# cloneofsimo/paint-with-words-sd

Measured on AMD Instinct MI355X. Metric: 512x512 images/sec (30 steps, CFG) SD1.5+PwW, higher is better.
Workload: dtype bf16

## Files before the change

### include/pww_hip_linear.h

```cpp
#ifndef PWW_HIP_LINEAR_H
#define PWW_HIP_LINEAR_H

#include "pww_hip.h"

#ifdef __cplusplus
extern "C" {
#endif

#define PWW_LINEAR_VERSION 100

int pww_linear_version(void);
const char *pww_linear_last_error(void);

#define PWW_LINEAR_NONE 0
#define PWW_LINEAR_BIAS 1
#define PWW_LINEAR_BIAS_RESIDUAL 2
#define PWW_LINEAR_BIAS_GEGLU 3
typedef struct pww_linear_desc {
    uint32_t size;
    int32_t dtype;
    int32_t M, N, K;
    int32_t epilogue;
    int64_t x_stride, y_stride, r_stride;
    int32_t tile_n, splitk;
} pww_linear_desc_t;
size_t pww_linear_workspace_bytes(const pww_linear_desc_t *desc);
int pww_linear_fwd(const void *x, const void *w, const void *bias, const void *residual, void *y, const pww_linear_desc_t *desc, void *workspace,
                   size_t workspace_bytes, void *stream);

#ifdef __cplusplus
}
#endif

#endif
```

### paint-with-words-sd_amd/build.py

```python
import os
import subprocess
import sys

HERE = os.path.dirname(os.path.abspath(__file__))
REPO = os.path.dirname(HERE)
CSRC = os.path.join(HERE, "csrc")
LIB = os.path.join(HERE, "pww_hip", "libpww_hip.so")
LIB_EXPERIMENTS = os.path.join(HERE, "pww_hip", "libpww_hip_experiments.so")
UNITS = [("pww_api.hip", [], ""), ("pww_attn.hip", [], ""), ("pww_cross.hip", [], ""), ("pww_cross_lean.hip", [], ""), ("pww_reduce.hip", [], ""),
         ("pww_mask.hip", [], ""), ("pww_qproj.hip", [], ""), ("pww_norm.hip", [], ""), ("pww_blocks.hip", [], ""), ("pww_conv.hip", [], ""), ("pww_probs.hip", [], ""),
         ("pww_attn_inst.hip", ["-DPWW_INST_F16"], ".f16"), ("pww_attn_inst.hip", ["-DPWW_INST_BF16"], ".bf16"),
         ("pww_cross_inst.hip", ["-DPWW_INST_F16", "-DPWW_INST_NW=2"], ".f16.nw2"), ("pww_cross_inst.hip", ["-DPWW_INST_F16", "-DPWW_INST_NW=4"], ".f16.nw4"),
         ("pww_cross_inst.hip", ["-DPWW_INST_BF16", "-DPWW_INST_NW=2"], ".bf16.nw2"), ("pww_cross_inst.hip", ["-DPWW_INST_BF16", "-DPWW_INST_NW=4"], ".bf16.nw4")]
EXPERIMENT_UNITS = [("pww_cross_out.hip", [], "")]
_ATTN_HEADERS = ["pww_tile.h", "pww_attn_core.h", "pww_cross_tile.h"]
SIDE_FLAGS = ["-fvisibility=hidden"]
SIDE_LIBS = {
    "long": ("pww_long.hip", _ATTN_HEADERS, "the long-prompt launches"),
    "scope": ("pww_scope.hip", _ATTN_HEADERS, "cross-attention with per-head / per-row score statistics"),
    "linear": ("pww_linear.hip", [], "linear layers with a bias / residual / GEGLU epilogue"),
    "regions": ("pww_regions.hip", [], "region masks and the per-pixel blend of the noise predictions"),
}
SOURCES = sorted({u[0] for u in UNITS + EXPERIMENT_UNITS})
HEADERS = ["pww_common.h", "pww_tile.h", "pww_attn_core.h", "pww_attn_kernel.h", "pww_cross_tile.h", "pww_cross_kernel.h", os.path.join(REPO, "include", "pww_hip.h")]
LIB_LONG, LIB_SCOPE, LIB_LINEAR, LIB_REGIONS = (os.path.join(HERE, "pww_hip", "libpww_hip_%s.so" % n) for n in SIDE_LIBS)
LONG_UNITS, SCOPE_UNITS, LINEAR_UNITS, REGIONS_UNITS = ([(v[0], SIDE_FLAGS, "")] for v in SIDE_LIBS.values())
HIPCC = os.environ.get("HIPCC", "/opt/rocm/bin/hipcc")
FLAGS = ["--offload-arch=gfx950", "-O3", "-std=c++17", "-fPIC", "-Wall",
         "-Wno-unused-function", "-mllvm", "-amdgpu-kernarg-preload-count=16"]


PER_FILE_FLAGS = {"pww_mask.hip": ["-ffp-contract=off"], "pww_regions.hip": ["-ffp-contract=off"]}


def _newer(target, deps):
    if not os.path.exists(target):
        return True
    t = os.path.getmtime(target)
    return any(os.path.getmtime(d) > t for d in deps)


def _deps():
    return ([os.path.join(CSRC, s) for s in SOURCES] + [h if os.path.isabs(h) else os.path.join(CSRC, h) for h in HEADERS] + [__file__])


def _build(lib, units, defines, objdir, verbose, jobs=None):
    os.makedirs(objdir, exist_ok=True)
# ... 79 lines not shown
```

### paint-with-words-sd_amd/csrc/pww_conv.hip

```cpp
#include "pww_common.h"

namespace pww {

namespace {

constexpr int CV_BM = 128, CV_THREADS = 256;
constexpr int CV_PF = 2;

__device__ __forceinline__ f32x4 mfma16(f16x8 a, f16x8 b, f32x4 c) { return __builtin_amdgcn_mfma_f32_16x16x32_f16(a, b, c, 0, 0, 0); }
__device__ __forceinline__ f32x4 mfma16(bf16x8 a, bf16x8 b, f32x4 c) { return __builtin_amdgcn_mfma_f32_16x16x32_bf16(a, b, c, 0, 0, 0); }

struct ConvCold {
    const void *bias, *residual;
    int nsplit, nslab;
};

__device__ __forceinline__ int xcd_remap(int orig, int nwg) {
    const int xcd = orig & 7, q = nwg >> 3, r = nwg & 7;
    return (xcd < r ? xcd * (q + 1) : r * (q + 1) + (xcd - r) * q) + (orig >> 3);
}

template <typename T>
__device__ __forceinline__ void epilogue4(const f32x4 &a, const ConvCold &cold, T *y, long off, int n) {
    typedef typename Vec<T>::v4 V4;
    V4 o;
#pragma unroll
    for (int j = 0; j < 4; ++j) o[j] = (T)a[j];
    if (cold.bias) {
        const V4 b = *reinterpret_cast<const V4 *>(reinterpret_cast<const T *>(cold.bias) + n);
#pragma unroll
        for (int j = 0; j < 4; ++j) o[j] = (T)((float)o[j] + (float)b[j]);
    }
    if (cold.residual) {
        const V4 r = *reinterpret_cast<const V4 *>(reinterpret_cast<const T *>(cold.residual) + off);
#pragma unroll
        for (int j = 0; j < 4; ++j) o[j] = (T)((float)r[j] + (float)o[j]);
    }
    *reinterpret_cast<V4 *>(y + off) = o;
}

template <typename T, int BN>
__global__ void __launch_bounds__(CV_THREADS, 2) conv3x3_kernel(const T *__restrict__ x, const T *__restrict__ w, void *__restrict__ out, int M, int N,
                                                            int Cin, int Hin, int Win, int Wo, int HWo, const ConvCold cold) {
    typedef typename Vec<T>::v8 V8;
    constexpr int BM = CV_BM, PF = CV_PF, XL = BM * 8 / CV_THREADS, WL = BN * 8 / CV_THREADS, RM = 4, RN = BN / 32;
    constexpr int XBYTES = BM * 128, STAGE = (BM + BN) * 128;
    __shared__ __attribute__((aligned(16))) char lds[2 * STAGE];

    const int geo = cold.nslab >> 24;
    const int nslab = cold.nslab & 0xffffff;
    const int stride = geo & 15, up = geo >> 4;
    const int Hv = Hin << up, Wv = Win << up;
    const int tid = threadIdx.x, lane = tid & 63, wave = tid >> 6, wm = wave >> 1, wn = wave & 1;
    const int ntm = (M + BM - 1) / BM;
    const int bid = xcd_remap(blockIdx.x, gridDim.x);
    const bool split = cold.nsplit > 1;
    const int tile = bid / cold.nsplit, ks = bid - tile * cold.nsplit;
    const int tm = tile % ntm, tn = tile / ntm;
    const int s_begin = (int)((long)ks * nslab / cold.nsplit), s_end = (int)((long)(ks + 1) * nslab / cold.nsplit);
    const int K9 = 9 * Cin;

// ... 90 lines not shown
        }
    }
#pragma unroll
    for (int t = 0; t < 2 * PF - 1; ++t) {
        if (i + t < n) {
            if (i + t + PF < n) load(t % PF);
            compute((i + t) & 1);
            if (i + t + 1 < n) store((t + 1) % PF, (i + t + 1) & 1);
            __syncthreads();
        }
    }

#pragma unroll
    for (int i = 0; i < RM; ++i) {
        const int m = tm * BM + wm * 64 + i * 16 + fr;
        if (m >= M) continue;
#pragma unroll
        for (int r = 0; r < RN; ++r) {
            const int n = tn * BN + wn * (BN / 2) + r * 16 + fq * 4;
            if (split) *reinterpret_cast<f32x4 *>(reinterpret_cast<float *>(out) + ((long)ks * M + m) * N + n) = acc[r][i];
            else epilogue4<T>(acc[r][i], cold, reinterpret_cast<T *>(out), (long)m * N + n, n);
        }
    }
}

template <typename T>
__global__ void __launch_bounds__(256) conv3x3_fold_kernel(const float *__restrict__ ws, T *__restrict__ y, long n4, int N, long MN, const ConvCold cold) {
    const long q = (long)blockIdx.x * 256 + threadIdx.x;
    if (q >= n4) return;
    const long off = q * 4;
    f32x4 a = *reinterpret_cast<const f32x4 *>(ws + off);
    for (int s = 1; s < cold.nsplit; ++s) a += *reinterpret_cast<const f32x4 *>(ws + s * MN + off);
    epilogue4<T>(a, cold, y, off, (int)(off % N));
}

struct ConvTune { int M, N, nslab, bn, nsplit; };
constexpr ConvTune CONV_TUNED[] = {
    {8192, 320, 45, 64, 3}, {8192, 320, 90, 64, 4}, {8192, 320, 135, 64, 3}, {8192, 640, 90, 128, 3},
    {2048, 320, 45, 64, 6}, {2048, 640, 45, 64, 3}, {2048, 640, 90, 128, 6}, {2048, 640, 135, 128, 6}, {2048, 640, 180, 128, 6},
    {2048, 640, 270, 128, 6}, {2048, 1280, 180, 128, 3},
    {512, 640, 90, 64, 6}, {512, 1280, 90, 128, 6}, {512, 1280, 180, 128, 12}, {512, 1280, 270, 128, 12}, {512, 1280, 360, 128, 12},
    {128, 1280, 180, 64, 12}, {128, 1280, 360, 64, 24},
    {65536, 640, 90, 128, 1}, {16384, 1280, 180, 128, 1},
    {4096, 640, 90, 128, 3}, {4096, 1280, 90, 128, 3}, {4096, 1280, 180, 128, 3}, {4096, 1280, 270, 128, 3}, {4096, 1280, 360, 128, 3},
    {1024, 1280, 180, 128, 6}, {1024, 1280, 360, 128, 6},
};

struct ConvPlan {
    int M, Ho, Wo, bn, nsplit, nslab, ntiles;
};

bool plan_conv(const pww_conv_desc_t *d, ConvPlan *p) {
    if (!d || d->size < sizeof(pww_conv_desc_t)) { set_error("conv3x3: descriptor missing or older than this library (size %u)", d ? d->size : 0u); return false; }
    const int up = d->upsample, s = d->stride;
    if ((d->dtype != PWW_DTYPE_F16 && d->dtype != PWW_DTYPE_BF16) || d->B < 1 || d->Hin < 1 || d->Win < 1 || d->Cin < 64 || d->Cin % 64 != 0
        || d->Cout < 64 || d->Cout % 64 != 0 || (s != 1 && s != 2) || (up != 0 && up != 1) || (up && s != 1) || d->Cin > 65536 || d->Cout > 65536) {
// ... 77 lines not shown
```

### paint-with-words-sd_amd/csrc/pww_linear.hip

```cpp
#define PWW_SIDE_LIB "libpww_hip_linear"
#include "pww_side_host.h"
#include "../../include/pww_hip_linear.h"

#define PWW_LINEAR_API extern "C" __attribute__((visibility("default")))

namespace pww {

namespace {

constexpr int LN_BM = 128, LN_THREADS = 256;
constexpr int LN_PF = 2;

__device__ __forceinline__ f32x4 mfma16(f16x8 a, f16x8 b, f32x4 c) { return __builtin_amdgcn_mfma_f32_16x16x32_f16(a, b, c, 0, 0, 0); }
__device__ __forceinline__ f32x4 mfma16(bf16x8 a, bf16x8 b, f32x4 c) { return __builtin_amdgcn_mfma_f32_16x16x32_bf16(a, b, c, 0, 0, 0); }

struct LinCold {
    const void *bias, *residual;
    long ys, rs;
    int nsplit, nslab, mode, inner;
};

__device__ __forceinline__ int xcd_remap(int orig, int nwg) {
    const int xcd = orig & 7, q = nwg >> 3, r = nwg & 7;
    return (xcd < r ? xcd * (q + 1) : r * (q + 1) + (xcd - r) * q) + (orig >> 3);
// ... 265 lines not shown
int linear_fwd(const void *x, const void *w, const void *bias, const void *residual, void *y, const pww_linear_desc_t *d, void *workspace,
               size_t workspace_bytes, hipStream_t stream) {
    LinPlan p;
    if (!plan_linear(d, &p)) return PWW_ENOTSUP;
    if (!x || !w || !y) { set_error("linear: x, w and y are required"); return PWW_EINVAL; }
    if ((d->epilogue >= PWW_LINEAR_BIAS && !bias) || (d->epilogue == PWW_LINEAR_BIAS_RESIDUAL && !residual)) {
        set_error("linear: epilogue %d needs its bias%s", d->epilogue, d->epilogue == PWW_LINEAR_BIAS_RESIDUAL ? " and residual" : "");
        return PWW_EINVAL;
    }
    if (!al16(x) || !al16(w) || !al16(y) || (reinterpret_cast<uintptr_t>(bias) & 7) || (reinterpret_cast<uintptr_t>(residual) & 7)) {
        set_error("linear: x, w, y must be 16-byte aligned, bias and residual 8-byte aligned");
        return PWW_EINVAL;
    }
    const size_t need = p.nsplit > 1 ? (size_t)p.nsplit * d->M * d->N * sizeof(float) : 0;
    if (need && (!workspace || !al16(workspace) || workspace_bytes < need)) {
        set_error("linear: split %d needs a 16-byte aligned workspace of %zu bytes (got %zu)", p.nsplit, need, workspace_bytes);
        return PWW_EINVAL;
    }
    if (!arch_ok()) return PWW_ENOTSUP;
    if (d->dtype == PWW_DTYPE_F16) return linear_launch<f16>(p, d, x, w, bias, residual, y, workspace, stream);
    return linear_launch<bf16>(p, d, x, w, bias, residual, y, workspace, stream);
}

}

PWW_LINEAR_API int pww_linear_version(void) { return PWW_LINEAR_VERSION; }
PWW_LINEAR_API const char *pww_linear_last_error(void) { return pww::last_error(); }
PWW_LINEAR_API size_t pww_linear_workspace_bytes(const pww_linear_desc_t *desc) { return pww::linear_workspace_bytes(desc); }
PWW_LINEAR_API int pww_linear_fwd(const void *x, const void *w, const void *bias, const void *residual, void *y, const pww_linear_desc_t *desc,
                                  void *workspace, size_t workspace_bytes, void *stream) {
    return pww::linear_fwd(x, w, bias, residual, y, desc, workspace, workspace_bytes, static_cast<hipStream_t>(stream));
}
```

### paint-with-words-sd_amd/pww_hip/_lib.py

```python
import ctypes
import os

_HERE = os.path.dirname(os.path.abspath(__file__))
LIB_PATH = os.environ.get("PWW_HIP_LIB", os.path.join(_HERE, "libpww_hip.so"))
EXPERIMENTS_LIB_PATH = os.environ.get("PWW_HIP_EXPERIMENTS_LIB", os.path.join(_HERE, "libpww_hip_experiments.so"))

LONG_LIB_PATH = os.environ.get("PWW_HIP_LONG_LIB", os.path.join(_HERE, "libpww_hip_long.so"))
SCOPE_LIB_PATH = os.environ.get("PWW_HIP_SCOPE_LIB", os.path.join(_HERE, "libpww_hip_scope.so"))
LINEAR_LIB_PATH = os.environ.get("PWW_HIP_LINEAR_LIB", os.path.join(_HERE, "libpww_hip_linear.so"))
REGIONS_LIB_PATH = os.environ.get("PWW_HIP_REGIONS_LIB", os.path.join(_HERE, "libpww_hip_regions.so"))

PWW_OK, PWW_EINVAL, PWW_ENOTSUP, PWW_EHIP = 0, -22, -95, -5
MIN_VERSION = 126
DTYPE_F16, DTYPE_BF16 = 0, 1
LAYOUT_NCHW, LAYOUT_NHWC = 0, 1
ACT_NONE, ACT_SILU = 0, 1
LINEAR_NONE, LINEAR_BIAS, LINEAR_BIAS_RESIDUAL, LINEAR_BIAS_GEGLU = 0, 1, 2, 3
MAX_HEAD_DIM = 160

EXPORTS = ("pww_version", "pww_has_experiments", "pww_last_error", "pww_device_arch", "pww_self_attn_fwd", "pww_cross_attn_fwd",
           "pww_cross_attn_fwd_stat", "pww_cross_attn_fwd_stat_ex",
           "pww_qk_reduce", "pww_mask_build", "pww_mask_build_rgb", "pww_mask_build_f32", "pww_resize_tokens", "pww_gauss_blur", "pww_inpaint_prep", "pww_cfg_combine", "pww_store_f32",
           "pww_workspace_bytes", "pww_profile_arm", "pww_profile_elapsed_us", "pww_profile_reset", "pww_debug_timeline", "pww_debug_path_counts",
           "pww_qproj_stat", "pww_qproj_parts", "pww_cross_attn_fwd_parts", "pww_mask_build_f32_levels", "pww_qk_parts", "pww_qk_parts_count",
           "pww_group_norm_fwd", "pww_group_norm_workspace_bytes", "pww_add_layer_norm", "pww_add_layer_norm_bias", "pww_geglu", "pww_bias_residual",
           "pww_conv3x3_workspace_bytes", "pww_conv3x3_fwd", "pww_cross_attn_probs")
EXPERIMENT_EXPORTS = ("pww_cross_attn_fwd_fused", "pww_cross_attn_fwd_fused_ex", "pww_cross_fused_workspace_bytes", "pww_cross_fused_state_bytes",
                      "pww_cross_attn_fwd_parts_out", "pww_cross_attn_out_supported")


LONG_EXPORTS = ("pww_long_version", "pww_long_last_error", "pww_long_qk_parts", "pww_long_qk_parts_count", "pww_long_cross_attn_fwd_parts",
                "pww_long_cross_attn_probs", "pww_long_profile_arm", "pww_long_profile_elapsed_us")
LONG_MIN_VERSION = 100
LONG_MIN_KEYS, LONG_MAX_KEYS = 129, 256


SCOPE_EXPORTS = ("pww_scope_version", "pww_scope_last_error", "pww_scope_head_parts_count", "pww_scope_head_parts", "pww_scope_cross_attn_fwd")
SCOPE_MIN_VERSION = 100
SCOPE_HEAD, SCOPE_ROW = 1, 2


LINEAR_EXPORTS = ("pww_linear_version", "pww_linear_last_error", "pww_linear_workspace_bytes", "pww_linear_fwd")
LINEAR_MIN_VERSION = 100


REGIONS_EXPORTS = ("pww_regions_version", "pww_regions_last_error", "pww_regions_masks", "pww_regions_combine")
REGIONS_MIN_VERSION = 100
REGIONS_MAX, REGIONS_MAX_PLANE, REGIONS_MAX_FEATHER = 8, 9216, 8.0


class AttnDesc(ctypes.Structure):
    _fields_ = [("dtype", ctypes.c_int32), ("B", ctypes.c_int32), ("H", ctypes.c_int32), ("N", ctypes.c_int32),
                ("M", ctypes.c_int32), ("D", ctypes.c_int32),
                ("q_stride", ctypes.c_int64 * 3), ("k_stride", ctypes.c_int64 * 3),
                ("v_stride", ctypes.c_int64 * 3), ("o_stride", ctypes.c_int64 * 3),
                ("scale", ctypes.c_float), ("bias_stride", ctypes.c_int64 * 4)]


class CrossOpts(ctypes.Structure):
    _fields_ = [("size", ctypes.c_uint32), ("bias_cols", ctypes.c_int32), ("coeff_scalar_dev", ctypes.c_void_p),
                ("bias_compact", ctypes.c_void_p), ("col_idx", ctypes.c_void_p), ("R", ctypes.c_int32), ("gated_images", ctypes.c_int32),
                ("compact_stride", ctypes.c_int64 * 2), ("col_idx_stride", ctypes.c_int64)]


class QprojDesc(ctypes.Structure):
# ... 161 lines not shown
    if not lib.pww_has_experiments():
        raise PwwHipError("%s was not built with -DPWW_EXPERIMENTS=1" % EXPERIMENTS_LIB_PATH)
    _exp = _bind(lib, True)
    return _exp


_P = ctypes.POINTER
_vp, _i32, _i64, _f32, _f64, _sz, _int = ctypes.c_void_p, ctypes.c_int32, ctypes.c_int64, ctypes.c_float, ctypes.c_double, ctypes.c_size_t, ctypes.c_int
_HINT = "(rebuild: python paint-with-words-sd_amd/build.py, or __graft_entry__.build())"
SIDE = {
    "long": dict(path="LONG_LIB_PATH", exports=LONG_EXPORTS, min_version=LONG_MIN_VERSION, missing_ok=False, needs="prompts longer than 77 tokens need it", sigs={
        "pww_long_qk_parts": ([_vp, _vp, _vp, _P(AttnDesc), _i32, _i32, _vp, _sz, _vp], _int),
        "pww_long_qk_parts_count": ([_P(AttnDesc)], _i32),
        "pww_long_cross_attn_fwd_parts": ([_vp, _vp, _vp, _vp, _vp, _i32, _f32, _vp, _P(AttnDesc), _vp, _i32, _vp, _P(CrossOpts), _vp], _int),
        "pww_long_cross_attn_probs": ([_vp, _vp, _vp, _vp, _i32, _f64, _f32, _vp, _P(AttnDesc), _P(CrossOpts), _vp, _P(ProbsDesc), _vp], _int),
        "pww_long_profile_arm": ([], _int),
        "pww_long_profile_elapsed_us": ([_P(_f32)], _int)}),
    "scope": dict(path="SCOPE_LIB_PATH", exports=SCOPE_EXPORTS, min_version=SCOPE_MIN_VERSION, missing_ok=True, needs="per-head / per-row score statistics need it", sigs={
        "pww_scope_head_parts_count": ([_P(AttnDesc)], _i32),
        "pww_scope_head_parts": ([_vp, _vp, _vp, _P(AttnDesc), _i32, _vp, _sz, _vp], _int),
        "pww_scope_cross_attn_fwd": ([_vp, _vp, _vp, _vp, _vp, _i32, _i32, _f32, _vp, _P(AttnDesc), _vp, _i32, _vp, _P(CrossOpts), _vp], _int)}),
    "linear": dict(path="LINEAR_LIB_PATH", exports=LINEAR_EXPORTS, min_version=LINEAR_MIN_VERSION, missing_ok=False, needs="linear layers on the native kernel need it", sigs={
        "pww_linear_workspace_bytes": ([_P(LinearDesc)], _sz),
        "pww_linear_fwd": ([_vp, _vp, _vp, _vp, _vp, _P(LinearDesc), _vp, _sz, _vp], _int)}),
    "regions": dict(path="REGIONS_LIB_PATH", exports=REGIONS_EXPORTS, min_version=REGIONS_MIN_VERSION, missing_ok=False, needs="region prompts need it", sigs={
        "pww_regions_masks": ([_vp, _i32, _i32, _vp, _i32, _f32, _vp, _vp], _int),
        "pww_regions_combine": ([_vp, _vp, _vp, _vp, _f32, _vp, _i32, _i32, _i32, _i64, _i32, _vp], _int)}),
}
_side = {}


def load_side(name):
    lib = _side.get(name)
    if lib is not None:
        return lib
    spec, path, so, pre = SIDE[name], globals()[SIDE[name]["path"]], "libpww_hip_%s.so" % name, "pww_%s_" % name
    if not os.path.isfile(path):
        if spec["missing_ok"]:
            return None
        raise PwwHipError("%s not found at %s: %s %s" % (so, path, spec["needs"], _HINT))
    try:
        lib = ctypes.CDLL(path)
        getattr(lib, pre + "version").restype = _int
        version = getattr(lib, pre + "version")()
    except (OSError, AttributeError) as e:
        raise PwwHipError("%s at %s cannot be loaded: %s %s" % (so, path, e, _HINT))
    if version // 100 != 1 or version < spec["min_version"]:
# ... 58 lines not shown
```

### paint-with-words-sd_amd/pww_hip/blocks.py

```python
import os
import types
import warnings

import torch
import torch.nn as nn
import torch.nn.functional as F

from . import ops

FUSED_NORM = os.environ.get("PWW_FUSED_NORM", "1") != "0"
BATCHED_TEMB = os.environ.get("PWW_BATCHED_TEMB", "1") != "0"
FOLD_CONV_BIAS = os.environ.get("PWW_FOLD_CONV_BIAS", "1") != "0"
CONV1X1_AS_LINEAR = os.environ.get("PWW_CONV1X1_AS_LINEAR", "1") != "0"
LINEAR = os.environ.get("PWW_LINEAR", "1")
CONV3X3 = os.environ.get("PWW_CONV3X3", "1") != "0"


_STATS = {k: [0, 0] for k in ("group_norm", "resnet_block", "transformer_block", "geglu", "conv1x1", "conv3x3", "linear")}
_UNRATED = ("conv1x1", "conv3x3", "linear")
_warned = set()


def stats():
    out = {k: {"fused": v[0], "declined": v[1]} for k, v in _STATS.items()}
    rated = [v for k, v in _STATS.items() if k not in _UNRATED]
    tot = sum(v[0] + v[1] for v in rated)
    out["hit_rate"] = (sum(v[0] for v in rated) / tot) if tot else None
    return out


def reset_stats():
    for v in _STATS.values():
        v[0] = v[1] = 0


def _count(op, fused, x=None, reason=None):
    _STATS[op][0 if fused else 1] += 1
    if not fused and FUSED_NORM and torch.is_tensor(x) and x.is_cuda and x.dtype in (torch.float16, torch.bfloat16):
# ... 89 lines not shown
        return out


def _conv_no_bias(conv, x):
    return F.conv2d(x, conv.weight, None, conv.stride, conv.padding, conv.dilation, conv.groups)


def _plain_conv(conv):
    return isinstance(conv, nn.Conv2d) and conv.bias is not None and conv.padding_mode == "zeros" and type(conv).forward is nn.Conv2d.forward \
        and "forward" not in conv.__dict__ and not conv._forward_hooks and not conv._forward_pre_hooks


def _resnet_forward(self, *args, **kwargs):
    covered = 1 <= len(args) <= 2 and set(kwargs) <= {"temb"} and not (len(args) == 2 and kwargs)
    input_tensor = args[0] if args else None
    if not covered or not _takes(input_tensor, self.norm1):
        _count("resnet_block", False, input_tensor, ("a call beyond (input_tensor, temb): %d positional, keywords %s" % (len(args), sorted(kwargs))) if not covered else _why_not(input_tensor))
        return self._pww_orig_forward(*args, **kwargs)
    temb = args[1] if len(args) == 2 else kwargs.get("temb")
    _count("resnet_block", True)
    fold = FOLD_CONV_BIAS and _plain_conv(self.conv1) and _plain_conv(self.conv2) and self.conv1.bias.dtype == input_tensor.dtype
    h = fused_group_norm(self.norm1, input_tensor, act="silu")
    if fold and _conv3x3_route(self.conv1, h):
        h = ops.conv3x3(h, self.conv1.weight)
    else:
        h = _conv_no_bias(self.conv1, h) if fold else self.conv1(h)
    add = None
    if temb is not None and getattr(self, "time_emb_proj", None) is not None:
        slot = self.__dict__.get("_pww_temb_slot")
        if slot is not None and temb.dtype == h.dtype and temb.dim() == 2 and not torch.is_grad_enabled():
            add = slot[0].project(temb)[:, slot[1]:slot[1] + slot[2]]
        else:
            add = self.time_emb_proj(F.silu(temb))
        if add.dtype != h.dtype:
            add = add.to(h.dtype)
    if fold and _takes(h, self.norm2):
        h = ops.group_norm(h, self.norm2.num_groups, self.norm2.weight, self.norm2.bias, self.norm2.eps, add=add, act="silu", pre_bias=self.conv1.bias)
    else:
        if fold:
            h = h + self.conv1.bias[None, :, None, None]
        h = fused_group_norm(self.norm2, h, add=add, act="silu")
    dropout = getattr(self, "dropout", None)
    if dropout is not None:
        h = dropout(h)
    if getattr(self, "conv_shortcut", None) is not None:
        input_tensor = self.conv_shortcut(input_tensor)
    scale = getattr(self, "output_scale_factor", 1.0)
    if fold and input_tensor.dtype == h.dtype and input_tensor.shape == (h.shape[0], self.conv2.out_channels) + h.shape[2:] and _conv3x3_route(self.conv2, h):
        out = ops.conv3x3(h, self.conv2.weight, self.conv2.bias, residual=input_tensor)
    elif fold and input_tensor.dtype == h.dtype and input_tensor.shape[1] % 8 == 0:
        out = ops.bias_residual(input_tensor, _conv_no_bias(self.conv2, h), self.conv2.bias)
    else:
        out = input_tensor + self.conv2(h)
    return out if scale == 1.0 else out / scale


def _is_conv3x3(m):
    return (isinstance(m, nn.Conv2d) and type(m).forward is nn.Conv2d.forward and m.kernel_size == (3, 3) and m.stride in ((1, 1), (2, 2))
            and m.padding == (1, 1) and m.dilation == (1, 1) and m.groups == 1 and m.padding_mode == "zeros")


STOCK_FROM_ROWS = 16384


def _conv3x3_route(conv, x, upsample=False):
    ok = (CONV3X3 and FUSED_NORM and torch.is_tensor(x) and x.dim() == 4 and _is_conv3x3(conv) and not torch.is_autocast_enabled() and not (torch.is_grad_enabled() and (x.requires_grad or conv.weight.requires_grad))
          and (conv.bias is None or conv.bias.dtype == x.dtype) and ops.conv3x3_takes(x, conv.weight, conv.stride[0], upsample)
          and (upsample or x.shape[0] * ((x.shape[2] - 1) // conv.stride[0] + 1) * ((x.shape[3] - 1) // conv.stride[0] + 1) < STOCK_FROM_ROWS))
    _STATS["conv3x3"][0 if ok else 1] += 1
    return ok


def _conv3x3_forward(self, x, *args, **kwargs):
    if not args and not kwargs and _conv3x3_route(self, x):
        return ops.conv3x3(x, self.weight, self.bias, stride=self.stride[0])
    return self._pww_orig_forward(x, *args, **kwargs)


def _upsample_conv(m):
    if getattr(m, "use_conv_transpose", False) or not getattr(m, "use_conv", True):
        return None
    conv = getattr(m, "Conv2d_0", None) if getattr(m, "name", "conv") != "conv" else getattr(m, "conv", None)
    return conv if _is_conv3x3(conv) and conv.stride == (1, 1) and "forward" not in conv.__dict__ and not conv._forward_hooks and not conv._forward_pre_hooks else None


def _upsample_forward(self, *args, **kwargs):
    plain = 1 <= len(args) <= 2 and set(kwargs) <= {"output_size"} and all(a is None for a in list(args[1:]) + list(kwargs.values()))
    x = args[0] if plain and not (len(args) == 2 and kwargs) else None
    conv = _upsample_conv(self)
    if x is not None and conv is not None and x.dim() == 4 and (getattr(self, "channels", None) in (None, x.shape[1])) and _conv3x3_route(conv, x, upsample=True):
        return ops.conv3x3(x, conv.weight, conv.bias, upsample=True)
    return self._pww_orig_forward(*args, **kwargs)


def _conv1x1_forward(self, x, *args, **kwargs):
    if (not args and not kwargs and FUSED_NORM and CONV1X1_AS_LINEAR and torch.is_tensor(x) and x.is_cuda and x.dim() == 4 and x.dtype == self.weight.dtype
            and x.shape[2] * x.shape[3] > 1 and x.is_contiguous(memory_format=torch.channels_last) and not torch.is_autocast_enabled()):
        B, C, H, W = x.shape
        _STATS["conv1x1"][0] += 1
        y = F.linear(x.permute(0, 2, 3, 1).reshape(B * H * W, C), self.weight.reshape(self.out_channels, C), self.bias)
        return y.view(B, H, W, self.out_channels).permute(0, 3, 1, 2)
    _STATS["conv1x1"][1] += 1
    return self._pww_orig_forward(x, *args, **kwargs)


def _is_conv1x1(m):
    return (isinstance(m, nn.Conv2d) and type(m).forward is nn.Conv2d.forward and m.kernel_size == (1, 1) and m.stride == (1, 1) and m.padding == (0, 0)
            and m.dilation == (1, 1) and m.groups == 1 and m.padding_mode == "zeros")


def _ln_takes(x, norm):
    return (FUSED_NORM and torch.is_tensor(x) and x.is_cuda and x.dtype in (torch.float16, torch.bfloat16) and x.dim() >= 2
            and len(norm.normalized_shape) == 1 and x.shape[-1] == norm.normalized_shape[0] and x.shape[-1] % 8 == 0 and x.shape[-1] <= 2048
            and (norm.weight is None or norm.weight.dtype == x.dtype) and not torch.is_autocast_enabled()
# ... 126 lines not shown
```

### paint-with-words-sd_amd/pww_hip/ops.py

```python
import ctypes

import torch

from . import _lib
from ._lib import AttnDesc, CrossOpts, ProbsDesc, QprojDesc, Region, PwwHipError

_DT = {torch.float16: _lib.DTYPE_F16, torch.bfloat16: _lib.DTYPE_BF16}


def _stream():
    return ctypes.c_void_p(torch.cuda.current_stream().cuda_stream)


def _ptr(t):
    return ctypes.c_void_p(t.data_ptr()) if t is not None else ctypes.c_void_p(0)


def _require_gpu(*tensors):
    for t in tensors:
        if t is not None and not t.is_cuda:
            raise PwwHipError("pww_hip ops need tensors on a HIP device (got %s); there is no CPU path" % t.device)


def _rows_ok(t):
# ... 888 lines not shown

def _khwc_weight(weight):
    if weight.is_contiguous(memory_format=torch.channels_last):
        return weight
    key = (weight.data_ptr(), weight._version, weight.dtype, weight.device)
    hit = weight.__dict__.get("_pww_khwc")
    if hit is not None and hit[0] == key:
        return hit[1]
    packed = weight.detach().permute(0, 2, 3, 1).contiguous()
    weight.__dict__["_pww_khwc"] = (key, packed)
    return packed


def conv3x3_takes(x, weight, stride=1, upsample=False):
    if not (torch.is_tensor(x) and x.is_cuda and x.dim() == 4 and x.dtype in _DT and torch.is_tensor(weight) and weight.dtype == x.dtype and weight.dim() == 4):
        return False
    B, C, H, W = x.shape
    Cout = weight.shape[0]
    return (tuple(weight.shape[1:]) == (C, 3, 3) and C % 64 == 0 and Cout % 64 == 0 and stride in (1, 2) and not (upsample and stride != 1)
            and x.is_contiguous(memory_format=torch.channels_last) and x.data_ptr() % 16 == 0
            and B * H * W * C < 2 ** 31 // 4)


def conv3x3(x, weight, bias=None, residual=None, stride=1, upsample=False, tile_n=0, splitk=0):
    _require_gpu(x, weight, bias, residual)
    if not conv3x3_takes(x, weight, stride, upsample):
        raise PwwHipError("conv3x3: needs a channels_last float16/bfloat16 x with Cin, Cout multiples of 64 and a 3 x 3 weight of its dtype")
    B, C, H, W = x.shape
    Cout = weight.shape[0]
    Hv, Wv = H << int(bool(upsample)), W << int(bool(upsample))
    Ho, Wo = (Hv - 1) // stride + 1, (Wv - 1) // stride + 1
    w = _khwc_weight(weight)
    if bias is not None and (bias.dtype != x.dtype or tuple(bias.shape) != (Cout,)):
        raise PwwHipError("conv3x3: bias must be a %s [%d]" % (x.dtype, Cout))
    if bias is not None:
        bias = bias.contiguous()
    if residual is not None:
        if tuple(residual.shape) != (B, Cout, Ho, Wo) or residual.dtype != x.dtype:
            raise PwwHipError("conv3x3: residual must be a %s %s" % (x.dtype, (B, Cout, Ho, Wo)))
        residual = residual.contiguous(memory_format=torch.channels_last)
    d = _lib.ConvDesc(ctypes.sizeof(_lib.ConvDesc), _DT[x.dtype], B, H, W, C, Cout, int(stride), int(bool(upsample)), int(tile_n), int(splitk), 0)
    lib = _lib.load()
    y = torch.empty((B, Cout, Ho, Wo), dtype=x.dtype, device=x.device, memory_format=torch.channels_last)
    nbytes = int(lib.pww_conv3x3_workspace_bytes(ctypes.byref(d)))
    ws = torch.empty(nbytes // 4, dtype=torch.float32, device=x.device) if nbytes else None
    with torch.cuda.device(x.device):
        _lib.check(lib.pww_conv3x3_fwd(_ptr(x), _ptr(w), _ptr(bias), _ptr(residual), _ptr(y), ctypes.byref(d), _ptr(ws), nbytes, _stream()), "pww_conv3x3_fwd")
    return y


def _linear_weight(weight):
    if not torch.is_tensor(weight) or weight.dim() not in (2, 4) or (weight.dim() == 4 and tuple(weight.shape[2:]) != (1, 1)):
        return None
    w = weight.detach().reshape(weight.shape[0], weight.shape[1]) if weight.dim() == 4 else weight.detach()
    return w if w.is_contiguous() and w.data_ptr() == weight.data_ptr() and w.data_ptr() % 16 == 0 else None


def linear_takes(x, weight, geglu=False, bias=None, residual=None, out=None):
    if not (torch.is_tensor(x) and x.is_cuda and x.dtype in _DT and x.dim() >= 2 and torch.is_tensor(weight) and weight.dtype == x.dtype):
        return False
    w = _linear_weight(weight)
    if w is None or x.shape[-1] != w.shape[1] or x.numel() == 0 or _rows(x, "linear") is None:
        return False
    N, K = w.shape
    rows, _, xs = _rows(x, "linear")
    if not (K % 64 == 0 and N % (128 if geglu else 64) == 0 and rows * xs < 2 ** 31 and rows * N < 2 ** 31 and N * K < 2 ** 31):
# ... 52 lines not shown
```

Measured before the change: 5.132.

## Add staged-row 3x3 convolution kernel reusing input rows across kx taps

Adds a new implicit-GEMM 3x3 conv kernel that stages a tile of 128+2 input pixel rows in LDS once per (ky, channel-block) and reuses it for all three kx taps, zeroing the left and right image edges in registers. Only the weights are reloaded per tap, which is meant to cut global input traffic and address math compared with the existing conv kernel. It comes with per-shape tuned tile widths and split-K factors, and is routed for the listed stride-1 SD1.5 UNet shapes. Upsample and stride-2 convs keep the old kernel. Adds code in the linear side library and a fallback path when the new kernel reports it is unsupported.

Measured after the change: 5.215, median of 6. 1.02x the previous value.

```diff
diff --git a/include/pww_hip_linear.h b/include/pww_hip_linear.h
--- a/include/pww_hip_linear.h
+++ b/include/pww_hip_linear.h
@@ -28,6 +28,18 @@
 int pww_linear_fwd(const void *x, const void *w, const void *bias, const void *residual, void *y, const pww_linear_desc_t *desc, void *workspace,
                    size_t workspace_bytes, void *stream);
 
+typedef struct pww_linear_conv_desc {
+    uint32_t size;
+    int32_t dtype;
+    int32_t B, Hin, Win, Cin, Cout;
+    int32_t stride, upsample;
+    int32_t tile_n, splitk;
+    int32_t _pad;
+} pww_linear_conv_desc_t;
+size_t pww_linear_conv3x3_workspace_bytes(const pww_linear_conv_desc_t *desc);
+int pww_linear_conv3x3_fwd(const void *x, const void *w, const void *bias, const void *residual, void *y, const pww_linear_conv_desc_t *desc,
+                           void *workspace, size_t workspace_bytes, void *stream);
+
 #ifdef __cplusplus
 }
 #endif
diff --git a/paint-with-words-sd_amd/build.py b/paint-with-words-sd_amd/build.py
--- a/paint-with-words-sd_amd/build.py
+++ b/paint-with-words-sd_amd/build.py
@@ -18,11 +18,11 @@
 SIDE_LIBS = {
     "long": ("pww_long.hip", _ATTN_HEADERS, "the long-prompt launches"),
     "scope": ("pww_scope.hip", _ATTN_HEADERS, "cross-attention with per-head / per-row score statistics"),
-    "linear": ("pww_linear.hip", [], "linear layers with a bias / residual / GEGLU epilogue"),
+    "linear": ("pww_linear.hip", ["pww_conv_rows.h", "pww_conv_fold.h"], "linear layers with a bias / residual / GEGLU epilogue; the staged-row 3 x 3 convolution"),
     "regions": ("pww_regions.hip", [], "region masks and the per-pixel blend of the noise predictions"),
 }
 SOURCES = sorted({u[0] for u in UNITS + EXPERIMENT_UNITS})
-HEADERS = ["pww_common.h", "pww_tile.h", "pww_attn_core.h", "pww_attn_kernel.h", "pww_cross_tile.h", "pww_cross_kernel.h", os.path.join(REPO, "include", "pww_hip.h")]
+HEADERS = ["pww_common.h", "pww_conv_fold.h", "pww_tile.h", "pww_attn_core.h", "pww_attn_kernel.h", "pww_cross_tile.h", "pww_cross_kernel.h", os.path.join(REPO, "include", "pww_hip.h")]
 LIB_LONG, LIB_SCOPE, LIB_LINEAR, LIB_REGIONS = (os.path.join(HERE, "pww_hip", "libpww_hip_%s.so" % n) for n in SIDE_LIBS)
 LONG_UNITS, SCOPE_UNITS, LINEAR_UNITS, REGIONS_UNITS = ([(v[0], SIDE_FLAGS, "")] for v in SIDE_LIBS.values())
 HIPCC = os.environ.get("HIPCC", "/opt/rocm/bin/hipcc")
diff --git a/paint-with-words-sd_amd/csrc/pww_conv.hip b/paint-with-words-sd_amd/csrc/pww_conv.hip
--- a/paint-with-words-sd_amd/csrc/pww_conv.hip
+++ b/paint-with-words-sd_amd/csrc/pww_conv.hip
@@ -10,33 +10,11 @@
 __device__ __forceinline__ f32x4 mfma16(f16x8 a, f16x8 b, f32x4 c) { return __builtin_amdgcn_mfma_f32_16x16x32_f16(a, b, c, 0, 0, 0); }
 __device__ __forceinline__ f32x4 mfma16(bf16x8 a, bf16x8 b, f32x4 c) { return __builtin_amdgcn_mfma_f32_16x16x32_bf16(a, b, c, 0, 0, 0); }
 
-struct ConvCold {
-    const void *bias, *residual;
-    int nsplit, nslab;
-};
+#include "pww_conv_fold.h"
 
 __device__ __forceinline__ int xcd_remap(int orig, int nwg) {
     const int xcd = orig & 7, q = nwg >> 3, r = nwg & 7;
     return (xcd < r ? xcd * (q + 1) : r * (q + 1) + (xcd - r) * q) + (orig >> 3);
-}
-
-template <typename T>
-__device__ __forceinline__ void epilogue4(const f32x4 &a, const ConvCold &cold, T *y, long off, int n) {
-    typedef typename Vec<T>::v4 V4;
-    V4 o;
-#pragma unroll
-    for (int j = 0; j < 4; ++j) o[j] = (T)a[j];
-    if (cold.bias) {
-        const V4 b = *reinterpret_cast<const V4 *>(reinterpret_cast<const T *>(cold.bias) + n);
-#pragma unroll
-        for (int j = 0; j < 4; ++j) o[j] = (T)((float)o[j] + (float)b[j]);
-    }
-    if (cold.residual) {
-        const V4 r = *reinterpret_cast<const V4 *>(reinterpret_cast<const T *>(cold.residual) + off);
-#pragma unroll
-        for (int j = 0; j < 4; ++j) o[j] = (T)((float)r[j] + (float)o[j]);
-    }
-    *reinterpret_cast<V4 *>(y + off) = o;
 }
 
 template <typename T, int BN>
@@ -173,16 +151,6 @@
             else epilogue4<T>(acc[r][i], cold, reinterpret_cast<T *>(out), (long)m * N + n, n);
         }
     }
-}
-
-template <typename T>
-__global__ void __launch_bounds__(256) conv3x3_fold_kernel(const float *__restrict__ ws, T *__restrict__ y, long n4, int N, long MN, const ConvCold cold) {
-    const long q = (long)blockIdx.x * 256 + threadIdx.x;
-    if (q >= n4) return;
-    const long off = q * 4;
-    f32x4 a = *reinterpret_cast<const f32x4 *>(ws + off);
-    for (int s = 1; s < cold.nsplit; ++s) a += *reinterpret_cast<const f32x4 *>(ws + s * MN + off);
-    epilogue4<T>(a, cold, y, off, (int)(off % N));
 }
 
 struct ConvTune { int M, N, nslab, bn, nsplit; };
diff --git a/paint-with-words-sd_amd/csrc/pww_conv_fold.h b/paint-with-words-sd_amd/csrc/pww_conv_fold.h
--- /dev/null
+++ b/paint-with-words-sd_amd/csrc/pww_conv_fold.h
@@ -0,0 +1,35 @@
+#pragma once
+
+struct ConvCold {
+    const void *bias, *residual;
+    int nsplit, nslab;
+};
+
+template <typename T>
+__device__ __forceinline__ void epilogue4(const f32x4 &a, const ConvCold &cold, T *y, long off, int n) {
+    typedef typename Vec<T>::v4 V4;
+    V4 o;
+#pragma unroll
+    for (int j = 0; j < 4; ++j) o[j] = (T)a[j];
+    if (cold.bias) {
+        const V4 b = *reinterpret_cast<const V4 *>(reinterpret_cast<const T *>(cold.bias) + n);
+#pragma unroll
+        for (int j = 0; j < 4; ++j) o[j] = (T)((float)o[j] + (float)b[j]);
+    }
+    if (cold.residual) {
+        const V4 r = *reinterpret_cast<const V4 *>(reinterpret_cast<const T *>(cold.residual) + off);
+#pragma unroll
+        for (int j = 0; j < 4; ++j) o[j] = (T)((float)r[j] + (float)o[j]);
+    }
+    *reinterpret_cast<V4 *>(y + off) = o;
+}
+
+template <typename T>
+__global__ void __launch_bounds__(256) conv3x3_fold_kernel(const float *__restrict__ ws, T *__restrict__ y, long n4, int N, long MN, const ConvCold cold) {
+    const long q = (long)blockIdx.x * 256 + threadIdx.x;
+    if (q >= n4) return;
+    const long off = q * 4;
+    f32x4 a = *reinterpret_cast<const f32x4 *>(ws + off);
+    for (int s = 1; s < cold.nsplit; ++s) a += *reinterpret_cast<const f32x4 *>(ws + s * MN + off);
+    epilogue4<T>(a, cold, y, off, (int)(off % N));
+}
diff --git a/paint-with-words-sd_amd/csrc/pww_conv_rows.h b/paint-with-words-sd_amd/csrc/pww_conv_rows.h
--- /dev/null
+++ b/paint-with-words-sd_amd/csrc/pww_conv_rows.h
@@ -0,0 +1,161 @@
+#pragma once
+#include "pww_conv_fold.h"
+
+constexpr int CR_BM = 128, CR_THREADS = 256, CR_XROWS = CR_BM + 2;
+
+template <typename T, int BN>
+__global__ void __launch_bounds__(CR_THREADS, 2) conv3x3_rows_kernel(const T *__restrict__ x, const T *__restrict__ w, void *__restrict__ out, int M, int N,
+                                                                     int Cin, int H, int W, const ConvCold cold) {
+    typedef typename Vec<T>::v8 V8;
+    constexpr int BM = CR_BM, XL = BM * 8 / CR_THREADS + 1, WL = BN * 8 / CR_THREADS, RM = 4, RN = BN / 32;
+    constexpr int XIMG = CR_XROWS * 128, WBYTES = BN * 128;
+    __shared__ __attribute__((aligned(16))) char lds[2 * XIMG + 2 * WBYTES];
+
+    const int tid = threadIdx.x, lane = tid & 63, wave = tid >> 6, wm = wave >> 1, wn = wave & 1;
+    const int ntm = (M + BM - 1) / BM;
+    const int bid = xcd_remap(blockIdx.x, gridDim.x);
+    const bool split = cold.nsplit > 1;
+    const int tile = bid / cold.nsplit, ks = bid - tile * cold.nsplit;
+    const int tm = tile % ntm, tn = tile / ntm;
+    const int g_begin = (int)((long)ks * cold.nslab / cold.nsplit), g_end = (int)((long)(ks + 1) * cold.nslab / cold.nsplit);
+    const int K9 = 9 * Cin, HW = H * W, nblk = Cin >> 6;
+
+    const int c = tid & 7;
+    int pbase[XL], oy[XL];
+#pragma unroll
+    for (int i = 0; i < XL; ++i) {
+        const int q = i < XL - 1 ? (tid >> 3) + 32 * i : BM + ((tid >> 3) & 1);
+        const int mc = tm * BM - 1 + q;
+        const bool in = mc >= 0 && mc < M;
+        const int m = in ? mc : 0;
+        const int rem = m % HW;
+        pbase[i] = m;
+        oy[i] = in ? rem / W : -4;
+    }
+    const T *wrow = w + (long)(tn * BN + (tid >> 3)) * K9 + c * 8;
+    const int swz = ((c ^ ((tid >> 3) & 7)) << 4);
+    const int swz_halo = ((c ^ ((tid >> 3) & 1)) << 4);
+
+    const int fr = lane & 15, fq = lane >> 4;
+    unsigned edge_l = 0, edge_r = 0;
+#pragma unroll
+    for (int q = 0; q < RM; ++q) {
+        const int ox = (tm * BM + wm * 64 + q * 16 + fr) % W;
+        edge_l |= (unsigned)(ox == 0) << q;
+        edge_r |= (unsigned)(ox == W - 1) << q;
+    }
+
+    u32x4 xr[XL], wr[2][WL];
+    unsigned xok = 0;
+    int x_ky = g_begin / nblk, x_ci = (g_begin - x_ky * nblk) << 6;
+    int w_ky = x_ky, w_ci = x_ci, w_kx = 0;
+    auto load_x = [&]() {
+        xok = 0;
+#pragma unroll
+        for (int i = 0; i < XL; ++i) {
+            const bool ok = (unsigned)(oy[i] + x_ky - 1) < (unsigned)H;
+            const int pix = ok ? pbase[i] + (x_ky - 1) * W : pbase[i];
+            xr[i] = *reinterpret_cast<const u32x4 *>(x + (unsigned)(pix * Cin + x_ci + c * 8));
+            xok |= (unsigned)ok << i;
+        }
+        x_ci += 64;
+        if (x_ci == Cin) { x_ci = 0; ++x_ky; }
+    };
+    auto load_w = [&](int p) {
+        const T *src = wrow + (w_ky * 3 + w_kx) * Cin + w_ci;
+#pragma unroll
+        for (int j = 0; j < WL; ++j) wr[p][j] = *reinterpret_cast<const u32x4 *>(src + (long)(32 * j) * K9);
+        if (++w_kx == 3) {
+            w_kx = 0;
+            w_ci += 64;
+            if (w_ci == Cin) { w_ci = 0; ++w_ky; }
+        }
+    };
+    auto store_x = [&](int img) {
+        char *base = lds + img * XIMG;
+        const u32x4 z = {0u, 0u, 0u, 0u};
+#pragma unroll
+        for (int i = 0; i < XL; ++i) asm volatile("" : "+v"(xr[i]));
+#pragma unroll
+        for (int i = 0; i < XL - 1; ++i) *reinterpret_cast<u32x4 *>(base + ((tid >> 3) + 32 * i) * 128 + swz) = (xok >> i) & 1u ? xr[i] : z;
+        if (tid < 16) *reinterpret_cast<u32x4 *>(base + (BM + (tid >> 3)) * 128 + swz_halo) = (xok >> (XL - 1)) & 1u ? xr[XL - 1] : z;
+    };
+    auto store_w = [&](int p, int buf) {
+        char *base = lds + 2 * XIMG + buf * WBYTES;
+#pragma unroll
+        for (int j = 0; j < WL; ++j) *reinterpret_cast<u32x4 *>(base + ((tid >> 3) + 32 * j) * 128 + swz) = wr[p][j];
+    };
+
+    f32x4 acc[RN][RM];
+#pragma unroll
+    for (int r = 0; r < RN; ++r)
+#pragma unroll
+        for (int i = 0; i < RM; ++i) acc[r][i] = f32x4{0.f, 0.f, 0.f, 0.f};
+
+    auto compute = [&](int img, int buf, int kx) {
+        const char *bx = lds + img * XIMG, *bw = lds + 2 * XIMG + buf * WBYTES;
+#pragma unroll
+        for (int kk = 0; kk < 2; ++kk) {
+            V8 xf[RM], wf[RN];
+#pragma unroll
+            for (int q = 0; q < RM; ++q) {
+                const int row = wm * 64 + q * 16 + fr + kx;
+                xf[q] = *reinterpret_cast<const V8 *>(bx + row * 128 + (((kk * 4 + fq) ^ (row & 7)) << 4));
+                if (kx == 0) xf[q] = (edge_l >> q) & 1u ? zero8<V8>() : xf[q];
+                if (kx == 2) xf[q] = (edge_r >> q) & 1u ? zero8<V8>() : xf[q];
+            }
+#pragma unroll
+            for (int r = 0; r < RN; ++r) {
+                const int row = wn * (BN / 2) + r * 16 + fr;
+                wf[r] = *reinterpret_cast<const V8 *>(bw + row * 128 + (((kk * 4 + fq) ^ (row & 7)) << 4));
+            }
+#pragma unroll
+            for (int r = 0; r < RN; ++r)
+#pragma unroll
+                for (int q = 0; q < RM; ++q) acc[r][q] = mfma16(wf[r], xf[q], acc[r][q]);
+        }
+    };
+
+    const int G = g_end - g_begin;
+    load_x();
+    load_w(0);
+    load_w(1);
+    store_x(0);
+    store_w(0, 0);
+    __syncthreads();
+    int g = 0;
+    for (; g + 3 <= G; g += 2) {
+#pragma unroll
+        for (int d = 0; d < 6; ++d) {
+            load_w(d & 1);
+            if (d % 3 == 0) load_x();
+            compute((d / 3) & 1, d & 1, d % 3);
+            store_w((d + 1) & 1, (d + 1) & 1);
+            if (d % 3 == 2) store_x(((d / 3) + 1) & 1);
+            __syncthreads();
+        }
+    }
+#pragma unroll
+    for (int d = 0; d < 6; ++d) {
+        if (g + d / 3 < G) {
+            if (g + (d + 2) / 3 < G) load_w(d & 1);
+            if (d % 3 == 0 && g + d / 3 + 1 < G) load_x();
+            compute((d / 3) & 1, d & 1, d % 3);
+            if (g + (d + 1) / 3 < G) store_w((d + 1) & 1, (d + 1) & 1);
+            if (d % 3 == 2 && g + d / 3 + 1 < G) store_x(((d / 3) + 1) & 1);
+            __syncthreads();
+        }
+    }
+
+#pragma unroll
+    for (int i = 0; i < RM; ++i) {
+        const int m = tm * BM + wm * 64 + i * 16 + fr;
+        if (m >= M) continue;
+#pragma unroll
+        for (int r = 0; r < RN; ++r) {
+            const int n = tn * BN + wn * (BN / 2) + r * 16 + fq * 4;
+            if (split) *reinterpret_cast<f32x4 *>(reinterpret_cast<float *>(out) + ((long)ks * M + m) * N + n) = acc[r][i];
+            else epilogue4<T>(acc[r][i], cold, reinterpret_cast<T *>(out), (long)m * N + n, n);
+        }
+    }
+}
diff --git a/paint-with-words-sd_amd/csrc/pww_linear.hip b/paint-with-words-sd_amd/csrc/pww_linear.hip
--- a/paint-with-words-sd_amd/csrc/pww_linear.hip
+++ b/paint-with-words-sd_amd/csrc/pww_linear.hip
@@ -311,6 +311,97 @@
     return linear_launch<bf16>(p, d, x, w, bias, residual, y, workspace, stream);
 }
 
+namespace {
+
+#include "pww_conv_rows.h"
+
+struct RowsTune { int M, N, Cin, bn, nsplit; };
+constexpr RowsTune ROWS_TUNED[] = {
+    {8192, 320, 320, 64, 1}, {8192, 320, 640, 64, 2}, {8192, 320, 960, 64, 3},
+    {2048, 640, 320, 64, 3}, {2048, 640, 640, 128, 6}, {2048, 640, 960, 128, 6}, {2048, 640, 1280, 128, 6}, {2048, 640, 1920, 128, 6},
+    {512, 1280, 640, 128, 6}, {512, 1280, 1280, 128, 12}, {512, 1280, 1920, 128, 12}, {512, 1280, 2560, 128, 12},
+    {128, 1280, 1280, 64, 12}, {128, 1280, 2560, 64, 24},
+};
+
+struct RowsPlan {
+    int M, bn, nsplit, ngroups, ntiles;
+};
+
+bool plan_rows(const pww_linear_conv_desc_t *d, RowsPlan *p) {
+    if (!d || d->size < sizeof(pww_linear_conv_desc_t)) { set_error("conv3x3 rows: descriptor missing or older than this library (size %u)", d ? d->size : 0u); return false; }
+    if ((d->dtype != PWW_DTYPE_F16 && d->dtype != PWW_DTYPE_BF16) || d->B < 1 || d->Hin < 1 || d->Win < 1 || d->Cin < 64 || d->Cin % 64 != 0
+        || d->Cout < 64 || d->Cout % 64 != 0 || d->stride != 1 || d->upsample != 0 || d->Cin > 65536 || d->Cout > 65536) {
+        set_error("conv3x3 rows: unsupported (dtype %d B %d %dx%d Cin %d Cout %d stride %d upsample %d): stride 1 without upsample, Cin and Cout "
+                  "multiples of 64", d->dtype, d->B, d->Hin, d->Win, d->Cin, d->Cout, d->stride, d->upsample);
+        return false;
+    }
+    const long M = (long)d->B * d->Hin * d->Win;
+    if (M * d->Cin >= (1L << 31) || M * d->Cout >= (1L << 31)) { set_error("conv3x3 rows: tensor of 2^31 elements or more"); return false; }
+    p->M = (int)M;
+    p->ngroups = 3 * d->Cin / 64;
+    const RowsTune *tuned = nullptr;
+    for (const RowsTune &t : ROWS_TUNED)
+        if (t.M == p->M && t.N == d->Cout && t.Cin == d->Cin) tuned = &t;
+    p->bn = d->tile_n ? d->tile_n : tuned ? tuned->bn : (d->Cout % 128 == 0 ? 128 : 64);
+    if ((p->bn != 64 && p->bn != 128) || d->Cout % p->bn != 0) { set_error("conv3x3 rows: tile_n %d does not divide Cout %d", d->tile_n, d->Cout); return false; }
+    p->ntiles = (p->M + CR_BM - 1) / CR_BM * (d->Cout / p->bn);
+    int ns = d->splitk;
+    if (ns <= 0 && tuned && p->bn == tuned->bn) ns = tuned->nsplit;
+    if (ns <= 0) {
+        ns = (480 + p->ntiles / 2) / p->ntiles;
+        if (ns > p->ngroups / 3) ns = p->ngroups / 3;
+        if (ns < 1) ns = 1;
+    }
+    if (ns > p->ngroups || ns > 64) { set_error("conv3x3 rows: split %d exceeds the %d K groups (or 64)", ns, p->ngroups); return false; }
+    p->nsplit = ns;
+    return true;
+}
+
+template <typename T>
+int rows_launch(const RowsPlan &p, const pww_linear_conv_desc_t *d, const void *x, const void *w, const void *bias, const void *residual, void *y, void *ws,
+                hipStream_t stream) {
+    ConvCold cold{bias, residual, p.nsplit, p.ngroups};
+    const T *xt = static_cast<const T *>(x), *wt = static_cast<const T *>(w);
+    const int N = d->Cout;
+    const dim3 grid(p.ntiles * p.nsplit), block(CR_THREADS);
+    void *out = p.nsplit == 1 ? y : ws;
+    if (p.bn == 128) launch_timed(conv3x3_rows_kernel<T, 128>, grid, block, 0, stream, xt, wt, out, p.M, N, d->Cin, d->Hin, d->Win, cold);
+    else launch_timed(conv3x3_rows_kernel<T, 64>, grid, block, 0, stream, xt, wt, out, p.M, N, d->Cin, d->Hin, d->Win, cold);
+    if (p.nsplit == 1) return check_hip(hipGetLastError(), "conv3x3 rows launch");
+    const long MN = (long)p.M * N, n4 = MN / 4;
+    launch_timed(conv3x3_fold_kernel<T>, dim3((unsigned)((n4 + 255) / 256)), dim3(256), 0, stream, static_cast<const float *>(ws), static_cast<T *>(y), n4,
+                 N, MN, cold);
+    return check_hip(hipGetLastError(), "conv3x3 rows fold launch");
+}
+
+}
+
+size_t rows_workspace_bytes(const pww_linear_conv_desc_t *d) {
+    RowsPlan p;
+    if (!plan_rows(d, &p)) return 0;
+    return p.nsplit > 1 ? (size_t)p.nsplit * p.M * d->Cout * sizeof(float) : 0;
+}
+
+int rows_fwd(const void *x, const void *w, const void *bias, const void *residual, void *y, const pww_linear_conv_desc_t *d, void *workspace,
+             size_t workspace_bytes, hipStream_t stream) {
+    RowsPlan p;
+    if (!plan_rows(d, &p)) return PWW_ENOTSUP;
+    if (!x || !w || !y) { set_error("conv3x3 rows: x, w and y are required"); return PWW_EINVAL; }
+    if (!al16(x) || !al16(w) || !al16(y) || (reinterpret_cast<uintptr_t>(bias) & 7) || (reinterpret_cast<uintptr_t>(residual) & 7)) {
+        set_error("conv3x3 rows: x, w, y must be 16-byte aligned, bias and residual 8-byte aligned");
+        return PWW_EINVAL;
+    }
+    const size_t need = p.nsplit > 1 ? (size_t)p.nsplit * p.M * d->Cout * sizeof(float) : 0;
+    if (need && (!workspace || !al16(workspace) || workspace_bytes < need)) {
+        set_error("conv3x3 rows: split %d needs a 16-byte aligned workspace of %zu bytes (got %zu)", p.nsplit, need, workspace_bytes);
+        return PWW_EINVAL;
+    }
+    if (!arch_ok()) return PWW_ENOTSUP;
+    if (d->dtype == PWW_DTYPE_F16) return rows_launch<f16>(p, d, x, w, bias, residual, y, workspace, stream);
+    return rows_launch<bf16>(p, d, x, w, bias, residual, y, workspace, stream);
+}
+
+
 }
 
 PWW_LINEAR_API int pww_linear_version(void) { return PWW_LINEAR_VERSION; }
@@ -320,3 +411,8 @@
                                   void *workspace, size_t workspace_bytes, void *stream) {
     return pww::linear_fwd(x, w, bias, residual, y, desc, workspace, workspace_bytes, static_cast<hipStream_t>(stream));
 }
+PWW_LINEAR_API size_t pww_linear_conv3x3_workspace_bytes(const pww_linear_conv_desc_t *desc) { return pww::rows_workspace_bytes(desc); }
+PWW_LINEAR_API int pww_linear_conv3x3_fwd(const void *x, const void *w, const void *bias, const void *residual, void *y, const pww_linear_conv_desc_t *desc,
+                                          void *workspace, size_t workspace_bytes, void *stream) {
+    return pww::rows_fwd(x, w, bias, residual, y, desc, workspace, workspace_bytes, static_cast<hipStream_t>(stream));
+}
diff --git a/paint-with-words-sd_amd/pww_hip/_lib.py b/paint-with-words-sd_amd/pww_hip/_lib.py
--- a/paint-with-words-sd_amd/pww_hip/_lib.py
+++ b/paint-with-words-sd_amd/pww_hip/_lib.py
@@ -40,7 +40,8 @@
 SCOPE_HEAD, SCOPE_ROW = 1, 2
 
 
-LINEAR_EXPORTS = ("pww_linear_version", "pww_linear_last_error", "pww_linear_workspace_bytes", "pww_linear_fwd")
+LINEAR_EXPORTS = ("pww_linear_version", "pww_linear_last_error", "pww_linear_workspace_bytes", "pww_linear_fwd",
+                  "pww_linear_conv3x3_workspace_bytes", "pww_linear_conv3x3_fwd")
 LINEAR_MIN_VERSION = 100
 
 
@@ -248,7 +249,9 @@
         "pww_scope_cross_attn_fwd": ([_vp, _vp, _vp, _vp, _vp, _i32, _i32, _f32, _vp, _P(AttnDesc), _vp, _i32, _vp, _P(CrossOpts), _vp], _int)}),
     "linear": dict(path="LINEAR_LIB_PATH", exports=LINEAR_EXPORTS, min_version=LINEAR_MIN_VERSION, missing_ok=False, needs="linear layers on the native kernel need it", sigs={
         "pww_linear_workspace_bytes": ([_P(LinearDesc)], _sz),
-        "pww_linear_fwd": ([_vp, _vp, _vp, _vp, _vp, _P(LinearDesc), _vp, _sz, _vp], _int)}),
+        "pww_linear_fwd": ([_vp, _vp, _vp, _vp, _vp, _P(LinearDesc), _vp, _sz, _vp], _int),
+        "pww_linear_conv3x3_workspace_bytes": ([_P(ConvDesc)], _sz),
+        "pww_linear_conv3x3_fwd": ([_vp, _vp, _vp, _vp, _vp, _P(ConvDesc), _vp, _sz, _vp], _int)}),
     "regions": dict(path="REGIONS_LIB_PATH", exports=REGIONS_EXPORTS, min_version=REGIONS_MIN_VERSION, missing_ok=False, needs="region prompts need it", sigs={
         "pww_regions_masks": ([_vp, _i32, _i32, _vp, _i32, _f32, _vp, _vp], _int),
         "pww_regions_combine": ([_vp, _vp, _vp, _vp, _f32, _vp, _i32, _i32, _i32, _i64, _i32, _vp], _int)}),
diff --git a/paint-with-words-sd_amd/pww_hip/blocks.py b/paint-with-words-sd_amd/pww_hip/blocks.py
--- a/paint-with-words-sd_amd/pww_hip/blocks.py
+++ b/paint-with-words-sd_amd/pww_hip/blocks.py
@@ -14,6 +14,7 @@
 CONV1X1_AS_LINEAR = os.environ.get("PWW_CONV1X1_AS_LINEAR", "1") != "0"
 LINEAR = os.environ.get("PWW_LINEAR", "1")
 CONV3X3 = os.environ.get("PWW_CONV3X3", "1") != "0"
+CONV3X3_ROWS = ops.CONV3X3_ROWS
 
 
 _STATS = {k: [0, 0] for k in ("group_norm", "resnet_block", "transformer_block", "geglu", "conv1x1", "conv3x3", "linear")}
@@ -149,7 +150,7 @@
     fold = FOLD_CONV_BIAS and _plain_conv(self.conv1) and _plain_conv(self.conv2) and self.conv1.bias.dtype == input_tensor.dtype
     h = fused_group_norm(self.norm1, input_tensor, act="silu")
     if fold and _conv3x3_route(self.conv1, h):
-        h = ops.conv3x3(h, self.conv1.weight)
+        h = ops.conv3x3(h, self.conv1.weight, rows=_conv3x3_rows(self.conv1, h))
     else:
         h = _conv_no_bias(self.conv1, h) if fold else self.conv1(h)
     add = None
@@ -174,7 +175,7 @@
         input_tensor = self.conv_shortcut(input_tensor)
     scale = getattr(self, "output_scale_factor", 1.0)
     if fold and input_tensor.dtype == h.dtype and input_tensor.shape == (h.shape[0], self.conv2.out_channels) + h.shape[2:] and _conv3x3_route(self.conv2, h):
-        out = ops.conv3x3(h, self.conv2.weight, self.conv2.bias, residual=input_tensor)
+        out = ops.conv3x3(h, self.conv2.weight, self.conv2.bias, residual=input_tensor, rows=_conv3x3_rows(self.conv2, h))
     elif fold and input_tensor.dtype == h.dtype and input_tensor.shape[1] % 8 == 0:
         out = ops.bias_residual(input_tensor, _conv_no_bias(self.conv2, h), self.conv2.bias)
     else:
@@ -188,6 +189,19 @@
 
 
 STOCK_FROM_ROWS = 16384
+
+
+CONV3X3_ROWS_ROUTES = frozenset([
+    (8192, 320, 320), (8192, 320, 640), (8192, 320, 960),
+    (2048, 640, 320), (2048, 640, 640), (2048, 640, 960), (2048, 640, 1280), (2048, 640, 1920),
+    (512, 1280, 640), (512, 1280, 1280), (512, 1280, 1920), (512, 1280, 2560),
+    (128, 1280, 1280), (128, 1280, 2560),
+])
+
+
+def _conv3x3_rows(conv, x):
+    listed = CONV3X3_ROWS and conv.stride == (1, 1) and (x.shape[0] * x.shape[2] * x.shape[3], conv.out_channels, conv.in_channels) in CONV3X3_ROWS_ROUTES
+    return None if listed else False
 
 
 def _conv3x3_route(conv, x, upsample=False):
@@ -200,7 +214,7 @@
 
 def _conv3x3_forward(self, x, *args, **kwargs):
     if not args and not kwargs and _conv3x3_route(self, x):
-        return ops.conv3x3(x, self.weight, self.bias, stride=self.stride[0])
+        return ops.conv3x3(x, self.weight, self.bias, stride=self.stride[0], rows=_conv3x3_rows(self, x))
     return self._pww_orig_forward(x, *args, **kwargs)
 
 
@@ -216,7 +230,7 @@
     x = args[0] if plain and not (len(args) == 2 and kwargs) else None
     conv = _upsample_conv(self)
     if x is not None and conv is not None and x.dim() == 4 and (getattr(self, "channels", None) in (None, x.shape[1])) and _conv3x3_route(conv, x, upsample=True):
-        return ops.conv3x3(x, conv.weight, conv.bias, upsample=True)
+        return ops.conv3x3(x, conv.weight, conv.bias, upsample=True, rows=False)
     return self._pww_orig_forward(*args, **kwargs)
 
 
diff --git a/paint-with-words-sd_amd/pww_hip/ops.py b/paint-with-words-sd_amd/pww_hip/ops.py
--- a/paint-with-words-sd_amd/pww_hip/ops.py
+++ b/paint-with-words-sd_amd/pww_hip/ops.py
@@ -1,4 +1,5 @@
 import ctypes
+import os
 
 import torch
 
@@ -934,7 +935,15 @@
             and B * H * W * C < 2 ** 31 // 4)
 
 
-def conv3x3(x, weight, bias=None, residual=None, stride=1, upsample=False, tile_n=0, splitk=0):
+CONV3X3_ROWS = os.environ.get("PWW_CONV3X3_ROWS", "1") != "0"
+
+
+def conv3x3_rows_takes(x, weight, stride=1, upsample=False, splitk=0, tile_n=0):
+    return (conv3x3_takes(x, weight, stride, upsample) and stride == 1 and not upsample and int(splitk) <= min(64, 3 * x.shape[1] // 64)
+            and (int(tile_n) == 0 or (int(tile_n) in (64, 128) and weight.shape[0] % int(tile_n) == 0)))
+
+
+def conv3x3(x, weight, bias=None, residual=None, stride=1, upsample=False, tile_n=0, splitk=0, rows=None):
     _require_gpu(x, weight, bias, residual)
     if not conv3x3_takes(x, weight, stride, upsample):
         raise PwwHipError("conv3x3: needs a channels_last float16/bfloat16 x with Cin, Cout multiples of 64 and a 3 x 3 weight of its dtype")
@@ -952,8 +961,17 @@
             raise PwwHipError("conv3x3: residual must be a %s %s" % (x.dtype, (B, Cout, Ho, Wo)))
         residual = residual.contiguous(memory_format=torch.channels_last)
     d = _lib.ConvDesc(ctypes.sizeof(_lib.ConvDesc), _DT[x.dtype], B, H, W, C, Cout, int(stride), int(bool(upsample)), int(tile_n), int(splitk), 0)
+    y = torch.empty((B, Cout, Ho, Wo), dtype=x.dtype, device=x.device, memory_format=torch.channels_last)
+    if rows or (rows is None and CONV3X3_ROWS and conv3x3_rows_takes(x, weight, stride, upsample, splitk, tile_n)):
+        lib = _lib.load_linear()
+        nbytes = int(lib.pww_linear_conv3x3_workspace_bytes(ctypes.byref(d)))
+        ws = torch.empty(nbytes // 4, dtype=torch.float32, device=x.device) if nbytes else None
+        with torch.cuda.device(x.device):
+            rc = lib.pww_linear_conv3x3_fwd(_ptr(x), _ptr(w), _ptr(bias), _ptr(residual), _ptr(y), ctypes.byref(d), _ptr(ws), nbytes, _stream())
+        if rows or rc != _lib.PWW_ENOTSUP:
+            _lib.check(rc, "pww_linear_conv3x3_fwd", lib)
+            return y
     lib = _lib.load()
-    y = torch.empty((B, Cout, Ho, Wo), dtype=x.dtype, device=x.device, memory_format=torch.channels_last)
     nbytes = int(lib.pww_conv3x3_workspace_bytes(ctypes.byref(d)))
     ws = torch.empty(nbytes // 4, dtype=torch.float32, device=x.device) if nbytes else None
     with torch.cuda.device(x.device):
```
